# GestaltCogTeam/STEP

Measured on AMD Instinct MI355X. Metric: training windows/sec on PEMS04, horizon-12 MAE parity, 1/2/4/8 MI355X, higher is better.
Workload: dtype f16 (TSFormer Q/K/weights) + bf16 (P, V, GraphWaveNet / graph-learner GEMMs) operands, f32 accumulate

## Files before the change

step_amd/build.py:

```python
import os
import subprocess
import sys

HERE = os.path.dirname(os.path.abspath(__file__))
CSRC = os.path.join(HERE, "csrc")
LIB = os.path.join(HERE, "libstep_hip.so")
SOURCES = ["errors.cpp", "comm.cpp", "gemm.hip", "gemm_bf16.hip", "tsformer_encoder.hip", "knn.hip", "selftest.hip",
           "dgl.hip", "dgl_conv_mfma.hip", "gwnet.hip", "optim.hip", "pretrain.hip", "pretrain_fused.hip", "pretrain_attn2.hip",
           "eval_cache.hip", "eval_metrics.hip", "train_tail.hip"]


def _newer(target, deps):
    if not os.path.exists(target):
        return True
    t = os.path.getmtime(target)
    return any(os.path.getmtime(d) > t for d in deps)


def build(force=False, verbose=True):
    hipcc = os.environ.get("HIPCC", "/opt/rocm/bin/hipcc")
    srcs = [os.path.join(CSRC, s) for s in SOURCES if os.path.exists(os.path.join(CSRC, s))]
    hdrs = [os.path.join(CSRC, f) for f in os.listdir(CSRC) if f.endswith(".h")]
    hdrs.append(os.path.join(HERE, "..", "include", "step_hip.h"))
    objs = []
    os.makedirs(os.path.join(HERE, "build"), exist_ok=True)
    procs = []
    for s in srcs:
        o = os.path.join(HERE, "build", os.path.basename(s) + ".o")
        objs.append(o)
        if force or _newer(o, [s] + hdrs):
            cmd = [hipcc, "--offload-arch=gfx950", "-O3", "-std=c++17", "-fPIC", "-x", "hip", "-c", s, "-o", o]
            if verbose:
                print(" ".join(cmd), flush=True)
            procs.append((s, subprocess.Popen(cmd, stdout=subprocess.PIPE, stderr=subprocess.STDOUT)))
    for s, p in procs:
        out, _ = p.communicate()
        if p.returncode != 0:
            sys.stderr.write(out.decode())
            raise RuntimeError("hipcc failed on " + s)
    if force or _newer(LIB, objs):
        cmd = [hipcc, "--offload-arch=gfx950", "-shared", "-fPIC", "-o", LIB] + objs + ["-ldl"]
        if verbose:
            print(" ".join(cmd), flush=True)
        subprocess.check_call(cmd)
    return LIB


if __name__ == "__main__":
    build(force="--force" in sys.argv)
```

step_amd/csrc/dgl.hip:

```cpp
#include "common.h"
#include "step_internal.h"

namespace {

constexpr int KW = 10;
constexpr int EMB = 100;

template <int CI, int CO, int TPT>
__global__ __launch_bounds__(256) void conv_relu_fwd_kernel(const float* __restrict__ in, const float* __restrict__ w,
                                                            const float* __restrict__ b, const float* __restrict__ in_sc,
                                                            const float* __restrict__ in_sh, float* __restrict__ out,
                                                            float* __restrict__ partial, int Tin, int stat_limit) {
    __shared__ __attribute__((aligned(16))) float ws[CI * KW * CO];
    __shared__ float red[4][2 * CO];
    const int tid = threadIdx.x, n = blockIdx.y;
    const int Tout = Tin - (KW - 1);
    for (int e = tid; e < CI * KW * CO; e += 256) {
        int co = e % CO, k = (e / CO) % KW, ci = e / (CO * KW);
        ws[e] = w[(co * CI + ci) * KW + k];
    }
    __syncthreads();
    const int t0 = (blockIdx.x * 256 + tid) * TPT;
    float acc[CO][TPT];
#pragma unroll
// ... 512 lines not shown
    if (tid < EMB) {
        drcv[(long)i * EMB + tid] = ra[tid] * sw[tid];
        atomicAdd(&dwcat[tid], rh[tid]);
        atomicAdd(&dwcat[EMB + tid], -rh[tid]);
    }
    if (tid == 0) {
        const float s = red[0] + red[1] + red[2] + red[3];
        atomicAdd(&dbcat[0], s);
        atomicAdd(&dbcat[1], -s);
    }
}
template <int VJ>
__global__ __launch_bounds__(256) void edge_bwd_col_kernel(const float* __restrict__ dz, const float* __restrict__ sndT,
                                                           const float* __restrict__ rcv, const float* __restrict__ wcat, int N,
                                                           float* __restrict__ dsndT) {
    const int lane = threadIdx.x & 63, wave = threadIdx.x >> 6;
    const int j = (blockIdx.x * 64 + lane) * VJ;
    const int f = blockIdx.y * 4 + wave;
    if (j >= N || f >= EMB) return;
    const float wd = wcat[f] - wcat[EMB + f];
    if constexpr (VJ == 4) {
        const float4 s4 = *(const float4*)(sndT + (long)f * N + j);
        float a0 = 0.f, a1 = 0.f, a2 = 0.f, a3 = 0.f;
#pragma unroll 8
        for (int i = 0; i < N; ++i) {
            const float r = rcv[(long)i * EMB + f];
            const float4 d = *(const float4*)(dz + (long)i * N + j);
            a0 += r + s4.x > 0.f ? d.x : 0.f; a1 += r + s4.y > 0.f ? d.y : 0.f;
            a2 += r + s4.z > 0.f ? d.z : 0.f; a3 += r + s4.w > 0.f ? d.w : 0.f;
        }
        *(float4*)(dsndT + (long)f * N + j) = make_float4(a0 * wd, a1 * wd, a2 * wd, a3 * wd);
    } else {
        const float s = sndT[(long)f * N + j];
        float a = 0.f;
#pragma unroll 8
        for (int i = 0; i < N; ++i) {
            float hid = rcv[(long)i * EMB + f] + s;
            float d = dz[(long)i * N + j];
            a += hid > 0.f ? d : 0.f;
        }
        dsndT[(long)f * N + j] = a * wd;
    }
}

__global__ void colsum_kernel(const float* __restrict__ x, long rows, int cols, long ld, float* __restrict__ out) {
    __shared__ float red[4][64];
    const int c = blockIdx.x * 64 + (threadIdx.x & 63);
    const int w = threadIdx.x >> 6;
    float s = 0.f;
    if (c < cols)
        for (long r = (long)blockIdx.y * 4 + w; r < rows; r += (long)gridDim.y * 4) s += x[r * ld + c];
    red[w][threadIdx.x & 63] = s;
    __syncthreads();
    if (w == 0 && c < cols) atomicAdd(&out[c], red[0][threadIdx.x] + red[1][threadIdx.x] + red[2][threadIdx.x] + red[3][threadIdx.x]);
}

}

int step_colsum_launch(const float* x, long rows, int cols, long ld, float* out, hipStream_t st) {
    int chunks = (int)((rows + 255) / 256);
    if (chunks > 512) chunks = 512;
    if (chunks < 1) chunks = 1;
    colsum_kernel<<<dim3(cdiv(cols, 64), chunks), 256, 0, st>>>(x, rows, cols, ld, out);
    STEP_LAUNCH_CHECK("colsum");
    return STEP_OK;
}

constexpr int DGL_SMALL = 256 + 64 + 1344 + 100 * 32;

__global__ void bn2_fused_coef_kernel(const float* __restrict__ dots, const float* __restrict__ stat, const float* __restrict__ gamma,
                                      double count, float* __restrict__ dgamma, float* __restrict__ dbeta, float* __restrict__ coef) {
    constexpr int C = 16;
    const int c = threadIdx.x;
    if (c >= C) return;
    const float S1 = dots[2 * c + 1];
    const float S2 = stat[3 * C + c] * (dots[2 * c] - stat[2 * C + c] * S1);
    dgamma[c] += S2;
    dbeta[c] += S1;
    coef[c] = (float)(S1 / count);
    coef[C + c] = (float)(S2 / count);
    coef[2 * C + c] = gamma[c] * stat[3 * C + c];
}

__global__ __launch_bounds__(256) void fc_prep_kernel(const float* __restrict__ fc_w, const float* __restrict__ st2, uint4* __restrict__ wp,
                                                      float* __restrict__ shiftdot, int T2) {
    __shared__ float red[4];
    const int o = blockIdx.y, t = blockIdx.x * 256 + threadIdx.x, tid = threadIdx.x;
    float acc = 0.f;
    if (t < T2) {
        float v[16];
#pragma unroll
        for (int c = 0; c < 16; ++c) v[c] = fc_w[((long)o * 16 + c) * T2 + t];
#pragma unroll
        for (int c = 0; c < 16; ++c) { acc += v[c] * st2[16 + c]; v[c] *= st2[c]; }
        uint4* dst = wp + ((long)o * T2 + t) * 2;
        dst[0] = make_uint4(pack_bf16x2(v[0], v[1]), pack_bf16x2(v[2], v[3]), pack_bf16x2(v[4], v[5]), pack_bf16x2(v[6], v[7]));
        dst[1] = make_uint4(pack_bf16x2(v[8], v[9]), pack_bf16x2(v[10], v[11]), pack_bf16x2(v[12], v[13]), pack_bf16x2(v[14], v[15]));
    }
    acc = wave_sum(acc);
    if ((tid & 63) == 0) red[tid >> 6] = acc;
    __syncthreads();
    if (tid == 0) atomicAdd(&shiftdot[o], red[0] + red[1] + red[2] + red[3]);
}
__global__ void gpre_init_kernel(float* __restrict__ gpre, const float* __restrict__ shiftdot, long n) {
    const long i = (long)blockIdx.x * 256 + threadIdx.x;
    if (i < n) gpre[i] = shiftdot[i % EMB];
}
__global__ __launch_bounds__(256) void fc_unpermute_kernel(const float* __restrict__ graw, const float* __restrict__ fc_w,
                                                           const float* __restrict__ st2, const float* __restrict__ colsum,
                                                           float* __restrict__ dfc_w, float* __restrict__ dots_o, int T2, int overwrite) {
    __shared__ float red[4][32];
    const int o = blockIdx.y, t = blockIdx.x * 256 + threadIdx.x, tid = threadIdx.x;
    const float cso = colsum[o];
    float d[32];
#pragma unroll
    for (int i = 0; i < 32; ++i) d[i] = 0.f;
    if (t < T2) {
        const float4* src = (const float4*)(graw + ((long)o * T2 + t) * 16);
        const float4 g0 = src[0], g1 = src[1], g2 = src[2], g3 = src[3];
        const float g[16] = {g0.x, g0.y, g0.z, g0.w, g1.x, g1.y, g1.z, g1.w, g2.x, g2.y, g2.z, g2.w, g3.x, g3.y, g3.z, g3.w};
        float w[16], old[16];
#pragma unroll
        for (int c = 0; c < 16; ++c) { const long idx = ((long)o * 16 + c) * T2 + t; w[c] = fc_w[idx]; old[c] = overwrite ? 0.f : dfc_w[idx]; }
#pragma unroll
        for (int c = 0; c < 16; ++c) {
            dfc_w[((long)o * 16 + c) * T2 + t] = old[c] + st2[c] * g[c] + st2[16 + c] * cso;
            d[2 * c] = w[c] * g[c]; d[2 * c + 1] = w[c] * cso;
        }
    }
#pragma unroll
    for (int i = 0; i < 32; ++i) {
        const float v = wave_sum(d[i]);
        if ((tid & 63) == 0) red[tid >> 6][i] = v;
    }
    __syncthreads();
    if (tid < 32) atomicAdd(&dots_o[o * 32 + tid], red[0][tid] + red[1][tid] + red[2][tid] + red[3][tid]);
}
__global__ void dots_reduce_kernel(const float* __restrict__ dots_o, float* __restrict__ dots) {
    const int i = threadIdx.x;
    if (i >= 32) return;
    double a = 0.0;
    for (int o = 0; o < EMB; ++o) a += dots_o[o * 32 + i];
    dots[i] = (float)a;
}

static bool dgl_channels_last(const StepDglParams* p) {
    const char* e = getenv("STEP_DGL_F32_STORAGE");
    return p->gemm_bf16 && !(e && e[0] == '1');
}

static bool dgl_legacy_bn_backward() {
    const char* e = getenv("STEP_DGL_LEGACY_BN");
    return e && e[0] == '1';
}

extern "C" long step_dgl_global_saved_floats(int N, int T) {
    long T1 = T - 9, T2 = T - 18;
    return (long)N * 8 * T1 + (long)N * 16 * T2 + (long)N * EMB + 4 * 8 + 4 * 16 + 4 * EMB + (long)EMB * 16 * T2 + 128;
}
static long fc_splitk_ws_floats(int N, int T2) {
    const int splits = step_gemm_auto_splitk(N, EMB, 16 * T2, 1);
    return splits > 1 ? (long)splits * N * EMB + 4 : 0;
}
extern "C" long step_dgl_global_work_floats(int N, int T, int backward) {
    long T1 = T - 9, T2 = T - 18;
    long nb1 = (long)N * cdiv(T1, 1024), nb2 = (long)N * cdiv(T2, 1024);
    long part = (nb1 > nb2 ? nb1 : nb2) * 32 + 64;
    if (!backward) return part + dgl_conv2_pack_floats() + 64 + fc_splitk_ws_floats(N, (int)T2);
    return part + (long)N * 16 * T2 + (long)N * 8 * T1 + (long)EMB * 16 * T2 + 2L * N * EMB + DGL_SMALL + dgl_conv2_wgrad_scratch_floats(N, (int)T1);
}

static float* saved_wp(float* saved, int N, int T) {
    long T1 = T - 9, T2 = T - 18;
    return saved + (long)N * 8 * T1 + (long)N * 16 * T2 + (long)N * EMB + 4 * 8 + 4 * 16 + 4 * EMB;
}
static void carve_saved(float* saved, int N, int T, float** a1, float** a2, float** gpre, float** st1, float** st2, float** st3) {
    long T1 = T - 9, T2 = T - 18;
    *a1 = saved; saved += (long)N * 8 * T1;
    *a2 = saved; saved += (long)N * 16 * T2;
    *gpre = saved; saved += (long)N * EMB;
    *st1 = saved; saved += 4 * 8;
    *st2 = saved; saved += 4 * 16;
    *st3 = saved;
}

static int dgl_bn_stats(const float* partial, int nblk, int C, double count, const float* gamma, const float* beta, float* rm, float* rv,
                        int training, float momentum, float* stat, double* sums, hipStream_t st) {
    if (nblk < 8192) {
        bn_finalize_kernel<<<C, 256, 0, st>>>(partial, nblk, C, count, gamma, beta, rm, rv, training, momentum, stat);
    } else {
        if (hipMemsetAsync(sums, 0, 2 * C * sizeof(double), st) != hipSuccess) { step_set_error("memset failed"); return STEP_ERR_HIP; }
        bn_sums_sliced_kernel<<<dim3(C, 32), 256, 0, st>>>(partial, nblk, C, sums);
        bn_finalize_sums_kernel<<<1, 64, 0, st>>>(sums, C, count, gamma, beta, rm, rv, training, momentum, stat);
    }
    STEP_LAUNCH_CHECK("bn_stats");
    return STEP_OK;
}

static int dgl_global_forward_impl(const float* series_nt, int N, int T, const StepDglParams* p, int training, float momentum,
                                   float* saved, float* work, double* sums, float* g, const StepDglShard* shard, int phase,
                                   hipStream_t st) {
    const int T1 = T - 9, T2 = T - 18;
    float *a1, *a2, *gpre, *st1, *st2, *st3;
    carve_saved(saved, N, T, &a1, &a2, &gpre, &st1, &st2, &st3);
    float* partial = work;
    const bool all = phase == 0;
    const double count1 = shard ? shard->count1 : (double)N * T1, count2 = shard ? shard->count2 : (double)N * T2;
    const bool cl = dgl_channels_last(p);
    const long part_floats = ((long)N * cdiv(T1, 1024) > (long)N * cdiv(T2, 1024) ? (long)N * cdiv(T1, 1024) : (long)N * cdiv(T2, 1024)) * 32 + 64;
    double* own_sums = (double*)(work + part_floats + dgl_conv2_pack_floats());
    float* wp = saved_wp(saved, N, T);
    float* shiftdot = wp + (long)EMB * 16 * T2;
    if (all || phase == 1) {
        int nblk;
        if (cl) {
            STEP_TRY(dgl_conv1_fwd_cl(series_nt, p->conv1_w, p->conv1_b, a1, partial, N, T, shard ? shard->own1 : T1, &nblk, st));
        } else {
            dim3 grid(cdiv(T1, 256 * 4), N);
            conv_relu_fwd_kernel<1, 8, 4><<<grid, 256, 0, st>>>(series_nt, p->conv1_w, p->conv1_b, nullptr, nullptr, a1, partial, T,
                                                                shard ? shard->own1 : T1);
            STEP_LAUNCH_CHECK("conv1");
            nblk = grid.x * grid.y;
        }
        if (shard) bn_sums_kernel<<<8, 256, 0, st>>>(partial, nblk, 8, sums);
        else STEP_TRY(dgl_bn_stats(partial, nblk, 8, count1, p->bn1_w, p->bn1_b, p->bn1_rm, p->bn1_rv, training, momentum, st1, own_sums, st));
        STEP_LAUNCH_CHECK("bn1");
    }
    if (all || phase == 2) {
        if (shard) bn_finalize_sums_kernel<<<1, 64, 0, st>>>(sums, 8, count1, p->bn1_w, p->bn1_b, p->bn1_rm, p->bn1_rv, training, momentum, st1);
        int nblk;
        if (cl) {
            STEP_TRY(dgl_conv2_fwd_cl(a1, p->conv2_w, p->conv2_b, st1, st1 + 8, a2, partial, N, T1, &nblk,
                                      work + part_floats, st));
        } else if (p->gemm_bf16) {
            STEP_TRY(dgl_conv2_fwd_mfma(a1, p->conv2_w, p->conv2_b, st1, st1 + 8, a2, partial, N, T1, &nblk, st));
        } else {
            dim3 grid(cdiv(T2, 256 * 4), N);
            conv_relu_fwd_kernel<8, 16, 4><<<grid, 256, 0, st>>>(a1, p->conv2_w, p->conv2_b, st1, st1 + 8, a2, partial, T1, T2);
            STEP_LAUNCH_CHECK("conv2");
            nblk = grid.x * grid.y;
        }
        if (shard) bn_sums_kernel<<<16, 256, 0, st>>>(partial, nblk, 16, sums + 16);
        else STEP_TRY(dgl_bn_stats(partial, nblk, 16, count2, p->bn2_w, p->bn2_b, p->bn2_rm, p->bn2_rv, training, momentum, st2, own_sums, st));
        STEP_LAUNCH_CHECK("bn2");
    }
    if (all || phase == 3) {
        if (shard) bn_finalize_sums_kernel<<<1, 64, 0, st>>>(sums + 16, 16, count2, p->bn2_w, p->bn2_b, p->bn2_rm, p->bn2_rv, training, momentum, st2);
        const long K = 16L * T2;
        StepGemm gm = gemm_desc(N, EMB, (int)K, a2, K, 1, p->fc_w, 1, K, gpre, EMB);
        if (cl) {
            if (hipMemsetAsync(shiftdot, 0, 128 * sizeof(float), st) != hipSuccess) { step_set_error("memset failed"); return STEP_ERR_HIP; }
            fc_prep_kernel<<<dim3(cdiv(T2, 256), EMB), 256, 0, st>>>(p->fc_w, st2, (uint4*)wp, shiftdot, T2);
            gpre_init_kernel<<<cdiv((long)N * EMB, 256), 256, 0, st>>>(gpre, shiftdot, (long)N * EMB);
            STEP_LAUNCH_CHECK("fc_prep");
            gm.a_bf16 = 1;
            gm.B = wp; gm.b_bf16 = 1;
        } else {
            if (hipMemsetAsync(gpre, 0, (size_t)N * EMB * sizeof(float), st) != hipSuccess) { step_set_error("memset failed"); return STEP_ERR_HIP; }
            gm.a_kscale = st2; gm.a_kshift = st2 + 16; gm.a_kperiod = T2;
        }
        gm.accumulate = 2;
        gm.splitk = -1;
        gm.compute_bf16 = p->gemm_bf16;
        if (fc_splitk_ws_floats(N, T2) > 0) {
            float* ws = work + part_floats + dgl_conv2_pack_floats() + 64;
            gm.splitk_ws = (float*)(((uintptr_t)ws + 15) & ~(uintptr_t)15);
            gm.splitk_ws_floats = fc_splitk_ws_floats(N, T2) - 4;
        }
        STEP_TRY(step_gemm_launch(gm, st));
    }
    if (all || phase == 4) {
        fc_post_bn3_kernel<<<EMB, 256, 0, st>>>(gpre, p->fc_b, N, p->bn3_w, p->bn3_b, p->bn3_rm, p->bn3_rv, training, momentum, st3, g);
        STEP_LAUNCH_CHECK("fc_post_bn3");
    }
    return STEP_OK;
}

extern "C" int step_dgl_global_forward(const float* series_nt, int N, int T, const StepDglParams* p, int training,
                                       float momentum, float* saved, float* work, float* g, void* stream) {
    STEP_REQUIRE(series_nt && p && saved && work && g && N > 0 && T > 18, "dgl_global_forward: bad arguments");
    return dgl_global_forward_impl(series_nt, N, T, p, training, momentum, saved, work, nullptr, g, nullptr, 0, (hipStream_t)stream);
}

extern "C" int step_dgl_global_forward_shard(const float* series_slice, int N, int Ts, const StepDglParams* p, int training,
                                             float momentum, float* saved, float* work, double* sums, float* g,
                                             const StepDglShard* shard, int phase, void* stream) {
    STEP_REQUIRE(series_slice && p && saved && work && sums && g && shard && N > 0 && Ts > 18 && phase >= 1 && phase <= 4,
                 "dgl_global_forward_shard: bad arguments");
    STEP_REQUIRE(shard->own1 > 0 && shard->own1 <= Ts - 9 && shard->count1 > 0 && shard->count2 > 0, "dgl_global_forward_shard: bad shard");
    return dgl_global_forward_impl(series_slice, N, Ts, p, training, momentum, saved, work, sums, g, shard, phase, (hipStream_t)stream);
}

extern "C" long step_dgl_global_offset(int N, int T, int item) {
    const long T1 = T - 9, T2 = T - 18;
    if (item == 0) return 0;
    if (item == 1) return (long)N * 8 * T1;
    if (item == 2) return (long)N * 8 * T1 + (long)N * 16 * T2;
    const long nb1 = (long)N * cdiv(T1, 1024), nb2 = (long)N * cdiv(T2, 1024);
    const long coef = (nb1 > nb2 ? nb1 : nb2) * 32 + 64 + (long)N * 16 * T2 + (long)N * 8 * T1 + (long)EMB * 16 * T2 + 2L * N * EMB;
    if (item == 10) return coef + 256;
    if (item == 11) return coef + 320;
    return -1;
}

static int dgl_global_backward_impl(const float* series_nt, int N, int T, const StepDglParams* p, const float* saved, const float* dg,
                                    float* work, const StepDglParams* grads, const StepDglShard* shard, int phase, void* stream);

extern "C" int step_dgl_global_backward(const float* series_nt, int N, int T, const StepDglParams* p, const float* saved,
                                        const float* dg, float* work, const StepDglParams* grads, void* stream) {
    return step_dgl_global_backward_phase(series_nt, N, T, p, saved, dg, work, grads, 0, stream);
}

extern "C" int step_dgl_global_backward_phase(const float* series_nt, int N, int T, const StepDglParams* p, const float* saved,
                                              const float* dg, float* work, const StepDglParams* grads, int phase, void* stream) {
    STEP_REQUIRE(series_nt && p && saved && dg && work && grads && N > 0 && T > 18 && (phase & ~STEP_DGL_FRESH_FC_GRAD) >= 0 &&
                 (phase & ~STEP_DGL_FRESH_FC_GRAD) <= 2, "dgl_global_backward: bad arguments");
    return dgl_global_backward_impl(series_nt, N, T, p, saved, dg, work, grads, nullptr, phase, stream);
}

extern "C" int step_dgl_global_backward_shard(const float* series_slice, int N, int Ts, const StepDglParams* p, const float* saved,
                                              const float* dg, float* work, const StepDglParams* grads, const StepDglShard* shard,
                                              int phase, void* stream) {
    const int ph = phase & ~STEP_DGL_FRESH_FC_GRAD;
    STEP_REQUIRE(series_slice && p && saved && dg && work && grads && shard && N > 0 && Ts > 18 && (ph == 1 || ph == 3 || ph == 4),
                 "dgl_global_backward_shard: bad arguments");
    STEP_REQUIRE(p->gemm_bf16 && Ts - 18 >= 128, "dgl_global_backward_shard: needs the bf16 contraction mode and a slice of >= 128 conv2 columns");
    return dgl_global_backward_impl(series_slice, N, Ts, p, saved, dg, work, grads, shard, phase, stream);
}

static int dgl_global_backward_impl(const float* series_nt, int N, int T, const StepDglParams* p, const float* saved, const float* dg,
                                    float* work, const StepDglParams* grads, const StepDglShard* shard, int phase, void* stream) {
    const int fresh_fc = (phase & STEP_DGL_FRESH_FC_GRAD) ? 1 : 0;
    phase &= ~STEP_DGL_FRESH_FC_GRAD;
    const bool do_fc = phase == 0 || phase == 1, do_mid = phase == 0 || phase == 2 || phase == 3, do_tail = phase == 0 || phase == 2 || phase == 4;
    hipStream_t st = (hipStream_t)stream;
    const int T1 = T - 9, T2 = T - 18;
    const long K = 16L * T2;
    float *a1, *a2, *gpre, *st1, *st2, *st3;
    carve_saved((float*)saved, N, T, &a1, &a2, &gpre, &st1, &st2, &st3);
    long nb1 = (long)N * cdiv(T1, 1024), nb2 = (long)N * cdiv(T2, 1024);
    float* partial = work;
    float* d_a2 = work + (nb1 > nb2 ? nb1 : nb2) * 32 + 64;
    float* d_a1 = d_a2 + (long)N * 16 * T2;
    float* wraw = d_a1 + (long)N * 8 * T1;
    float* dgpre = wraw + (long)EMB * K;
    float* dgpreT = dgpre + (long)N * EMB;
    float* coef = dgpreT + (long)N * EMB;
    float* dots = coef + 256;
    float* graw = coef + 320;
    float* wg_scratch = coef + DGL_SMALL;
    const bool fuse2 = T2 >= 128 && (shard || !dgl_legacy_bn_backward());
    const double count1 = shard ? shard->count1 : (double)N * T1, count2 = shard ? shard->count2 : (double)N * T2;
    if (dgl_channels_last(p)) {
        const float* wp = saved_wp((float*)saved, N, T);
        float* dots_o = coef + 256 + 64 + 1344;
        float* colsum = coef + 128;
        if (do_fc) {
            bn3_relu_bwd_kernel<<<EMB, 256, 0, st>>>(dg, gpre, N, p->bn3_w, st3, grads->bn3_w, grads->bn3_b, grads->fc_b, dgpre, dgpreT, colsum);
            STEP_LAUNCH_CHECK("bn3_bwd");
            StepGemm gm = gemm_desc(EMB, (int)K, N, dgpre, 1, EMB, a2, K, 1, wraw, K);
            gm.b_bf16 = 1;
            gm.compute_bf16 = 1;
            STEP_TRY(step_gemm_launch(gm, st));
            if (hipMemsetAsync(dots_o, 0, EMB * 32 * sizeof(float), st) != hipSuccess) { step_set_error("memset failed"); return STEP_ERR_HIP; }
            fc_unpermute_kernel<<<dim3(cdiv(T2, 256), EMB), 256, 0, st>>>(wraw, p->fc_w, st2, colsum, grads->fc_w, dots_o, T2, fresh_fc);
            dots_reduce_kernel<<<1, 64, 0, st>>>(dots_o, dots);
            STEP_LAUNCH_CHECK("fc_unpermute");
        }
        if (do_mid) {
            bn2_fused_coef_kernel<<<1, 64, 0, st>>>(dots, st2, p->bn2_w, count2, grads->bn2_w, grads->bn2_b, coef);
            STEP_LAUNCH_CHECK("bn2_fused_coef");
            StepGemm gm = gemm_desc(N, (int)K, EMB, dgpre, EMB, 1, wp, K, 1, d_a2, K);
            gm.b_bf16 = 1;
            gm.compute_bf16 = 1;
            GemmFused fu = {nullptr, nullptr, a2, coef, st2, 16, T2, GEMM_FUSED_INTERLEAVED};
            STEP_TRY(step_gemm_launch_fused(gm, fu, st));
            STEP_TRY(dgl_conv2_wgrad_cl(d_a2, a1, wg_scratch, graw, N, T1, st));
        }
        if (do_tail) {
            STEP_TRY(dgl_conv2_wgrad_finish(graw, p->conv2_w, st1, p->bn1_w, p->bn1_b, count1, grads->conv2_w, grads->conv2_b, grads->bn1_w,
                                            grads->bn1_b, coef + 64, 1, st));
            STEP_TRY(dgl_conv2_dgrad_cl(d_a2, p->conv2_w, st1, d_a1, N, T1, a1, coef + 64, st1, shard ? shard->own1 : T1, wraw, st));
            STEP_TRY(dgl_conv1_wgrad_cl(d_a1, series_nt, wg_scratch, grads->conv1_w, grads->conv1_b, N, T, st));
        }
        return STEP_OK;
    }
    if (do_fc) {
        float* colsum = coef + 128;
        bn3_relu_bwd_kernel<<<EMB, 256, 0, st>>>(dg, gpre, N, p->bn3_w, st3, grads->bn3_w, grads->bn3_b, grads->fc_b, dgpre, dgpreT, colsum);
        STEP_LAUNCH_CHECK("bn3_bwd");
        {
            StepGemm gm = gemm_desc(EMB, (int)K, N, dgpre, 1, EMB, a2, K, 1, grads->fc_w, K);
            gm.accumulate = fresh_fc ? 0 : 1;
            gm.c_nscale = st2; gm.c_nshift = st2 + 16; gm.c_nperiod = T2; gm.c_mvec = colsum;
            gm.compute_bf16 = p->gemm_bf16;
            if (fuse2) {
                if (hipMemsetAsync(dots, 0, 32 * sizeof(float), st) != hipSuccess) { step_set_error("memset failed"); return STEP_ERR_HIP; }
                GemmFused fu = {p->fc_w, dots, nullptr, nullptr, nullptr, 16, T2};
                STEP_TRY(step_gemm_launch_fused(gm, fu, st));
            } else {
                STEP_TRY(step_gemm_launch(gm, st));
            }
        }
    }
    if (!do_mid && !do_tail) return STEP_OK;
    if (do_mid) {
        StepGemm gm = gemm_desc(N, (int)K, EMB, dgpreT, 1, N, p->fc_w, K, 1, d_a2, K);
        if (p->gemm_bf16 || fuse2) { gm.A = dgpre; gm.sam = EMB; gm.sak = 1; }
        gm.compute_bf16 = p->gemm_bf16;
        if (fuse2) {
            bn2_fused_coef_kernel<<<1, 64, 0, st>>>(dots, st2, p->bn2_w, count2, grads->bn2_w, grads->bn2_b, coef);
            STEP_LAUNCH_CHECK("bn2_fused_coef");
            GemmFused fu = {nullptr, nullptr, a2, coef, st2, 16, T2};
            STEP_TRY(step_gemm_launch_fused(gm, fu, st));
        } else {
            STEP_TRY(step_gemm_launch(gm, st));
        }
    }
    if (do_mid && !fuse2) {
        dim3 grid(cdiv(T2, 1024), 16, N);
        bn_bwd_reduce_kernel<16><<<grid, 256, 0, st>>>(d_a2, a2, st2, T2, partial);
        STEP_LAUNCH_CHECK("bn2_bwd_reduce");
        bn_bwd_finalize_kernel<<<16, 256, 0, st>>>(partial, (int)nb2, 16, (double)N * T2, p->bn2_w, st2, grads->bn2_w, grads->bn2_b, coef);
        STEP_LAUNCH_CHECK("bn2_bwd_finalize");
        bn_bwd_apply_kernel<16><<<grid, 256, 0, st>>>(d_a2, a2, st2, coef, T2);
        STEP_LAUNCH_CHECK("bn2_bwd_apply");
    }
    const bool fuse1 = p->gemm_bf16 && (shard || !dgl_legacy_bn_backward());
    if (fuse1) {
        if (do_mid) STEP_TRY(dgl_conv2_wgrad_xhat_mfma(d_a2, a1, st1, wg_scratch, graw, N, T1, st));
        if (!do_tail) return STEP_OK;
        STEP_TRY(dgl_conv2_wgrad_finish(graw, p->conv2_w, st1, p->bn1_w, p->bn1_b, count1, grads->conv2_w, grads->conv2_b, grads->bn1_w,
                                        grads->bn1_b, coef + 64, 0, st));
        STEP_TRY(dgl_conv2_dgrad_mfma(d_a2, p->conv2_w, d_a1, N, T1, a1, coef + 64, st1, shard ? shard->own1 : T1, st));
    } else if (p->gemm_bf16) {
        STEP_TRY(dgl_conv2_wgrad_mfma(d_a2, a1, st1, st1 + 8, wg_scratch, grads->conv2_w, grads->conv2_b, N, T1, st));
        STEP_TRY(dgl_conv2_dgrad_mfma(d_a2, p->conv2_w, d_a1, N, T1, nullptr, nullptr, nullptr, T1, st));
    } else {
        conv_bwd_weight_kernel<8, 16><<<N, 256, 0, st>>>(d_a2, a1, st1, st1 + 8, grads->conv2_w, grads->conv2_b, T1);
        STEP_LAUNCH_CHECK("conv2_bwd_weight");
        conv_bwd_data_kernel<8, 16, 4><<<dim3(cdiv(T1, 1024), N), 256, 0, st>>>(d_a2, p->conv2_w, d_a1, T1);
        STEP_LAUNCH_CHECK("conv2_bwd_data");
    }
    if (!fuse1) {
        dim3 grid(cdiv(T1, 1024), 8, N);
        bn_bwd_reduce_kernel<8><<<grid, 256, 0, st>>>(d_a1, a1, st1, T1, partial);
        STEP_LAUNCH_CHECK("bn1_bwd_reduce");
        bn_bwd_finalize_kernel<<<8, 256, 0, st>>>(partial, (int)nb1, 8, (double)N * T1, p->bn1_w, st1, grads->bn1_w, grads->bn1_b, coef);
        STEP_LAUNCH_CHECK("bn1_bwd_finalize");
        bn_bwd_apply_kernel<8><<<grid, 256, 0, st>>>(d_a1, a1, st1, coef, T1);
        STEP_LAUNCH_CHECK("bn1_bwd_apply");
    }
    if (p->gemm_bf16) {
        STEP_TRY(dgl_conv1_wgrad_mfma(d_a1, series_nt, wg_scratch, grads->conv1_w, grads->conv1_b, N, T, st));
    } else {
        conv_bwd_weight_kernel<1, 8><<<N, 256, 0, st>>>(d_a1, series_nt, nullptr, nullptr, grads->conv1_w, grads->conv1_b, T);
        STEP_LAUNCH_CHECK("conv1_bwd_weight");
    }
    return STEP_OK;
}

extern "C" long step_dgl_edges_saved_floats(int B, int N) { return 2L * N * EMB + (long)N * N + 2L * B * N * N; }
extern "C" long step_dgl_edges_theta_offset(int N) { return 2L * N * EMB + (long)N * N; }

extern "C" int step_dgl_edges_forward(const float* g, int N, int B, const StepDglParams* p, const float* u, uint64_t seed,
                                      float temperature, float* saved, float* theta_out, float* adj_out, void* stream) {
    return step_dgl_edges_forward_dyn(g, N, B, p, u, seed, temperature, saved, theta_out, adj_out, nullptr, stream);
}
extern "C" int step_dgl_edges_forward_dyn(const float* g, int N, int B, const StepDglParams* p, const float* u, uint64_t seed,
                                          float temperature, float* saved, float* theta_out, float* adj_out, const StepDynState* dyn,
                                          void* stream) {
    STEP_REQUIRE(g && p && saved && adj_out && N > 0 && B > 0 && temperature > 0.f, "dgl_edges_forward: bad arguments");
    hipStream_t st = (hipStream_t)stream;
    float* sndT = saved;
    float* rcv = sndT + (long)N * EMB;
    float* z = rcv + (long)N * EMB;
    float* theta = z + (long)N * N;
    float* y0 = theta + (long)B * N * N;
    StepGemm gs = gemm_desc(N, EMB, EMB, g, EMB, 1, p->fc_out_w, 1, 2 * EMB, sndT, 1);
    gs.scn = N;
    STEP_TRY(step_gemm_launch(gs, st));
    StepGemm gr = gemm_desc(N, EMB, EMB, g, EMB, 1, p->fc_out_w + EMB, 1, 2 * EMB, rcv, EMB);
    gr.bias = p->fc_out_b;
    STEP_TRY(step_gemm_launch(gr, st));
    {
        const int vec4 = N % 4 == 0 && N >= 1024 && (((uintptr_t)sndT | (uintptr_t)z) & 15) == 0;
        edge_logit_kernel<<<dim3(cdiv(N, vec4 ? 1024 : 256), N), 256, 0, st>>>(sndT, rcv, p->fc_cat_w, p->fc_cat_b, N, z, vec4);
    }
    STEP_LAUNCH_CHECK("edge_logit");
    int gx = cdiv((long)N * N, 256);
    if (gx > 4096) gx = 4096;
    gumbel_sample_kernel<<<dim3(gx, B), 256, 0, st>>>(z, u, B, N, (uint32_t)seed, (uint32_t)(seed >> 32), 1.f / temperature, theta, y0, adj_out, dyn);
    STEP_LAUNCH_CHECK("gumbel_sample");
    if (theta_out && theta_out != theta) {
        if (hipMemcpyAsync(theta_out, theta, (size_t)B * N * N * sizeof(float), hipMemcpyDeviceToDevice, st) != hipSuccess) {
            step_set_error("dgl_edges_forward: theta copy failed");
            return STEP_ERR_HIP;
        }
    }
    return STEP_OK;
}

extern "C" long step_dgl_edges_work_floats(int N) { return (long)N * N + 2L * N * EMB; }

extern "C" int step_dgl_edges_backward(const float* g, int N, int B, const StepDglParams* p, const float* saved,
                                       const float* dtheta, const float* dadj, float temperature, float* work,
                                       const StepDglParams* grads, float* dg, void* aux_stream, void* stream) {
    STEP_REQUIRE(g && p && saved && work && grads && dg && N > 0 && B > 0, "dgl_edges_backward: bad arguments");
    hipStream_t st = (hipStream_t)stream;
    AuxLane lane(st, (hipStream_t)aux_stream);
    const float* sndT = saved;
    const float* rcv = sndT + (long)N * EMB;
    const float* theta = rcv + (long)N * EMB + (long)N * N;
    const float* y0 = theta + (long)B * N * N;
    float* dz = work;
    float* drcv = dz + (long)N * N;
    float* dsndT = drcv + (long)N * EMB;
    int gx = cdiv((long)N * N, 256);
    if (gx > 4096) gx = 4096;
    edge_dz_kernel<<<gx, 256, 0, st>>>(dtheta, dadj, theta, y0, B, N, 1.f / temperature, dz);
// ... 25 lines not shown
```

step_amd/csrc/step_internal.h:

```cpp
#pragma once
#include <hip/hip_runtime.h>
#include <vector>
#include "../../include/step_hip.h"

enum { GEMM_FUSED_INTERLEAVED = 1, GEMM_FUSED_FFN_FWD = 2, GEMM_FUSED_MASKNZ = 4, GEMM_FUSED_BF16OUT = 8 };
struct GemmFused {
    const float* dotw; float* dots;
    const float* bnx; const float* bncoef; const float* bnstat;
    int channels, period;
    int flags;
    const float* ffn_bias; const void* maskx; float p; unsigned seed_lo, seed_hi, site;
};

struct GemmKSeg { long a_off, b_off, a_bs, b_bs; int a_rs, b_rs; };
constexpr int GEMM_KSEG_MAX = 128;
int step_gemm_segmented_launch(StepGemm g, const GemmKSeg* ktab, int ktab_per, hipStream_t st);

int step_gemm_launch(StepGemm g, hipStream_t st);
int step_gemm_auto_splitk(int M, int N, int K, int batch);
int step_gemm_launch_fused(StepGemm g, const GemmFused& fused, hipStream_t st);
int step_gemm_bf16_launch(StepGemm g, hipStream_t st, const GemmFused* fused = nullptr);
int step_gemm_f32_fast_launch(StepGemm g, hipStream_t st, const GemmFused* fused = nullptr);

static inline StepGemm gemm_desc(int M, int N, int K, const float* A, long sam, long sak, const float* B, long sbk,
                                 long sbn, float* C, long ldc) {
    StepGemm g;
    memset(&g, 0, sizeof(g));
    g.M = M; g.N = N; g.K = K; g.batch = 1;
    g.A = A; g.sam = sam; g.sak = sak;
    g.B = B; g.sbk = sbk; g.sbn = sbn;
    g.C = C; g.ldc = ldc; g.scn = 1;
    g.alpha = 1.f; g.splitk = 1;
    return g;
}

int step_gemm_rowsum_separate(StepGemm* g, hipStream_t st);
int dgl_conv2_fwd_mfma(const float* a1, const float* w, const float* b, const float* sc, const float* sh, float* a2, float* partial,
                       int N, int T1, int* nblk, hipStream_t st);
int dgl_conv2_dgrad_mfma(const float* dz, const float* w, float* din, int N, int T1, const float* bnx, const float* coef, const float* stat,
                         int own, hipStream_t st);
int dgl_conv2_wgrad_xhat_mfma(const float* dz, const float* a1, const float* stat1, float* scratch, float* graw, int N, int T1, hipStream_t st);
int dgl_conv2_wgrad_finish(const float* graw, const float* w, const float* stat1, const float* gamma1, const float* beta1, double count,
                           float* dw, float* db, float* dgamma1, float* dbeta1, float* coef1, int raw, hipStream_t st);
int dgl_conv1_fwd_cl(const float* x, const float* w, const float* b, void* a1h, float* partial, int N, int T, int stat_limit, int* nblk,
                     hipStream_t st);
long dgl_conv2_pack_floats();
int dgl_conv2_fwd_cl(const void* a1h, const float* w, const float* b, const float* sc, const float* sh, void* a2h, float* partial, int N,
                     int T1, int* nblk, float* pack, hipStream_t st);
int dgl_conv2_dgrad_cl(const void* dz2h, const float* w, const float* sc, void* dz1h, int N, int T1, const void* a1h, const float* coef,
                       const float* stat, int own, float* pack, hipStream_t st);
int dgl_conv2_wgrad_cl(const void* dz2h, const void* a1h, float* scratch, float* graw, int N, int T1, hipStream_t st);
int dgl_conv1_wgrad_cl(const void* dz1h, const float* x, float* scratch, float* dw, float* db, int N, int T, hipStream_t st);
long dgl_conv2_wgrad_scratch_floats(int N, int T1);
int dgl_conv2_wgrad_mfma(const float* dz, const float* a1, const float* sc, const float* sh, float* scratch, float* dw, float* db, int N,
                         int T1, hipStream_t st);
int dgl_conv1_wgrad_mfma(const float* dz, const float* x, float* scratch, float* dw, float* db, int N, int T, hipStream_t st);
int step_colsum_launch(const float* x, long rows, int cols, long ld, float* out, hipStream_t st);

struct AuxLane {
    hipStream_t main, aux;
    bool on;
    int next = 0, base = 0;
    AuxLane(hipStream_t m, hipStream_t a, int base_ = 0) : main(m), aux(a), on(a != nullptr && a != m), base(base_) {}
    static hipEvent_t event(int k) {
        thread_local std::vector<hipEvent_t> pool[16];
        int dev = 0;
        (void)hipGetDevice(&dev);
        std::vector<hipEvent_t>& v = pool[dev & 15];
        while ((int)v.size() <= k) {
            hipEvent_t e;
            if (hipEventCreateWithFlags(&e, hipEventDisableTiming) != hipSuccess) return nullptr;
            v.push_back(e);
        }
        return v[k];
    }
    hipStream_t fork() {
        if (!on) return main;
        hipEvent_t e = event(base + (next++ & 63));
        if (!e || hipEventRecord(e, main) != hipSuccess || hipStreamWaitEvent(aux, e, 0) != hipSuccess) { on = false; return main; }
        return aux;
    }
    hipEvent_t mark() {
        if (!on) return nullptr;
        hipEvent_t e = event(base + (next++ & 63));
        if (!e || hipEventRecord(e, main) != hipSuccess) { on = false; return nullptr; }
        return e;
    }
    hipStream_t after(hipEvent_t e) {
        if (!on || !e) return main;
        if (hipStreamWaitEvent(aux, e, 0) != hipSuccess) { on = false; return main; }
        return aux;
    }
    hipEvent_t done() {
        if (!on) return nullptr;
        hipEvent_t e = event(base + (next++ & 63));
        if (!e || hipEventRecord(e, aux) != hipSuccess) return nullptr;
        return e;
    }
    int wait_done(hipEvent_t e) {
        if (!on) return STEP_OK;
        if (!e) return join();
        if (hipStreamWaitEvent(main, e, 0) != hipSuccess) { step_set_error("backward: stream join failed"); return STEP_ERR_HIP; }
        return STEP_OK;
    }
    int join() {
        if (!on) return STEP_OK;
        hipEvent_t e = event(base + (next++ & 63));
        if (!e || hipEventRecord(e, aux) != hipSuccess || hipStreamWaitEvent(main, e, 0) != hipSuccess) {
            step_set_error("backward: stream join failed");
            return STEP_ERR_HIP;
        }
        return STEP_OK;
    }
};
```

Before: 2358.

## Fuse graph-learner FC weight-gradient GEMM with unpermute and BN dot reduction

Adds a dedicated MFMA kernel for the graph-learner FC weight gradient. Its epilogue applies the BN2 scale/shift, writes dfc_w in the original layout and produces the per-channel dot partials in one pass. This replaces the generic GEMM, the raw-gradient buffer round trip, the unpermute kernel and the memset. It also adds an opt-in fused forward kernel that folds the weight pack/scale into a split-K MFMA GEMM. The forward path stays behind an environment flag, while the backward fused path is on by default. The cost is a new hand-written kernel, and the per-block LDS and partial workspace (passed via wraw) need to be large enough.

```diff
diff --git a/step_amd/build.py b/step_amd/build.py
--- a/step_amd/build.py
+++ b/step_amd/build.py
@@ -6,7 +6,7 @@
 CSRC = os.path.join(HERE, "csrc")
 LIB = os.path.join(HERE, "libstep_hip.so")
 SOURCES = ["errors.cpp", "comm.cpp", "gemm.hip", "gemm_bf16.hip", "tsformer_encoder.hip", "knn.hip", "selftest.hip",
-           "dgl.hip", "dgl_conv_mfma.hip", "gwnet.hip", "optim.hip", "pretrain.hip", "pretrain_fused.hip", "pretrain_attn2.hip",
+           "dgl.hip", "dgl_fc.hip", "dgl_conv_mfma.hip", "gwnet.hip", "optim.hip", "pretrain.hip", "pretrain_fused.hip", "pretrain_attn2.hip",
            "eval_cache.hip", "eval_metrics.hip", "train_tail.hip"]
 
 
diff --git a/step_amd/csrc/dgl.hip b/step_amd/csrc/dgl.hip
--- a/step_amd/csrc/dgl.hip
+++ b/step_amd/csrc/dgl.hip
@@ -688,6 +688,15 @@
 static bool dgl_legacy_bn_backward() {
     const char* e = getenv("STEP_DGL_LEGACY_BN");
     return e && e[0] == '1';
+}
+
+static bool dgl_fc_staged() {
+    const char* e = getenv("STEP_DGL_FC_STAGED");
+    return e && e[0] == '1';
+}
+static bool dgl_fc_fwd_fused() {
+    const char* e = getenv("STEP_DGL_FC_FWD_FUSED");
+    return e && e[0] == '1' && !dgl_fc_staged();
 }
 
 extern "C" long step_dgl_global_saved_floats(int N, int T) {
@@ -783,27 +792,35 @@
     if (all || phase == 3) {
         if (shard) bn_finalize_sums_kernel<<<1, 64, 0, st>>>(sums + 16, 16, count2, p->bn2_w, p->bn2_b, p->bn2_rm, p->bn2_rv, training, momentum, st2);
         const long K = 16L * T2;
-        StepGemm gm = gemm_desc(N, EMB, (int)K, a2, K, 1, p->fc_w, 1, K, gpre, EMB);
-        if (cl) {
-            if (hipMemsetAsync(shiftdot, 0, 128 * sizeof(float), st) != hipSuccess) { step_set_error("memset failed"); return STEP_ERR_HIP; }
-            fc_prep_kernel<<<dim3(cdiv(T2, 256), EMB), 256, 0, st>>>(p->fc_w, st2, (uint4*)wp, shiftdot, T2);
-            gpre_init_kernel<<<cdiv((long)N * EMB, 256), 256, 0, st>>>(gpre, shiftdot, (long)N * EMB);
-            STEP_LAUNCH_CHECK("fc_prep");
-            gm.a_bf16 = 1;
-            gm.B = wp; gm.b_bf16 = 1;
+        if (cl && dgl_fc_fwd_fused() && dgl_fc_fwd_cl_ok(N, a2, wp)) {
+            const int splits = step_gemm_auto_splitk(N, EMB, (int)K, 1), ksteps = cdiv(K, 64);
+            const int tper = 4 * cdiv(ksteps, splits > 1 ? splits : 1);
+            float* ws = work + part_floats + dgl_conv2_pack_floats() + 64;
+            ws = (float*)(((uintptr_t)ws + 15) & ~(uintptr_t)15);
+            STEP_TRY(dgl_fc_fwd_cl(a2, p->fc_w, st2, wp, ws, gpre, N, T2, tper, st));
         } else {
-            if (hipMemsetAsync(gpre, 0, (size_t)N * EMB * sizeof(float), st) != hipSuccess) { step_set_error("memset failed"); return STEP_ERR_HIP; }
-            gm.a_kscale = st2; gm.a_kshift = st2 + 16; gm.a_kperiod = T2;
-        }
-        gm.accumulate = 2;
-        gm.splitk = -1;
-        gm.compute_bf16 = p->gemm_bf16;
-        if (fc_splitk_ws_floats(N, T2) > 0) {
-            float* ws = work + part_floats + dgl_conv2_pack_floats() + 64;
-            gm.splitk_ws = (float*)(((uintptr_t)ws + 15) & ~(uintptr_t)15);
-            gm.splitk_ws_floats = fc_splitk_ws_floats(N, T2) - 4;
-        }
-        STEP_TRY(step_gemm_launch(gm, st));
+            StepGemm gm = gemm_desc(N, EMB, (int)K, a2, K, 1, p->fc_w, 1, K, gpre, EMB);
+            if (cl) {
+                if (hipMemsetAsync(shiftdot, 0, 128 * sizeof(float), st) != hipSuccess) { step_set_error("memset failed"); return STEP_ERR_HIP; }
+                fc_prep_kernel<<<dim3(cdiv(T2, 256), EMB), 256, 0, st>>>(p->fc_w, st2, (uint4*)wp, shiftdot, T2);
+                gpre_init_kernel<<<cdiv((long)N * EMB, 256), 256, 0, st>>>(gpre, shiftdot, (long)N * EMB);
+                STEP_LAUNCH_CHECK("fc_prep");
+                gm.a_bf16 = 1;
+                gm.B = wp; gm.b_bf16 = 1;
+            } else {
+                if (hipMemsetAsync(gpre, 0, (size_t)N * EMB * sizeof(float), st) != hipSuccess) { step_set_error("memset failed"); return STEP_ERR_HIP; }
+                gm.a_kscale = st2; gm.a_kshift = st2 + 16; gm.a_kperiod = T2;
+            }
+            gm.accumulate = 2;
+            gm.splitk = -1;
+            gm.compute_bf16 = p->gemm_bf16;
+            if (fc_splitk_ws_floats(N, T2) > 0) {
+                float* ws = work + part_floats + dgl_conv2_pack_floats() + 64;
+                gm.splitk_ws = (float*)(((uintptr_t)ws + 15) & ~(uintptr_t)15);
+                gm.splitk_ws_floats = fc_splitk_ws_floats(N, T2) - 4;
+            }
+            STEP_TRY(step_gemm_launch(gm, st));
+        }
     }
     if (all || phase == 4) {
         fc_post_bn3_kernel<<<EMB, 256, 0, st>>>(gpre, p->fc_b, N, p->bn3_w, p->bn3_b, p->bn3_rm, p->bn3_rv, training, momentum, st3, g);
@@ -894,14 +911,18 @@
         if (do_fc) {
             bn3_relu_bwd_kernel<<<EMB, 256, 0, st>>>(dg, gpre, N, p->bn3_w, st3, grads->bn3_w, grads->bn3_b, grads->fc_b, dgpre, dgpreT, colsum);
             STEP_LAUNCH_CHECK("bn3_bwd");
-            StepGemm gm = gemm_desc(EMB, (int)K, N, dgpre, 1, EMB, a2, K, 1, wraw, K);
-            gm.b_bf16 = 1;
-            gm.compute_bf16 = 1;
-            STEP_TRY(step_gemm_launch(gm, st));
-            if (hipMemsetAsync(dots_o, 0, EMB * 32 * sizeof(float), st) != hipSuccess) { step_set_error("memset failed"); return STEP_ERR_HIP; }
-            fc_unpermute_kernel<<<dim3(cdiv(T2, 256), EMB), 256, 0, st>>>(wraw, p->fc_w, st2, colsum, grads->fc_w, dots_o, T2, fresh_fc);
-            dots_reduce_kernel<<<1, 64, 0, st>>>(dots_o, dots);
-            STEP_LAUNCH_CHECK("fc_unpermute");
+            if (!dgl_fc_staged()) {
+                STEP_TRY(dgl_fc_wgrad_cl(dgpre, a2, p->fc_w, st2, colsum, grads->fc_w, wraw, dots, N, T2, fresh_fc, st));
+            } else {
+                StepGemm gm = gemm_desc(EMB, (int)K, N, dgpre, 1, EMB, a2, K, 1, wraw, K);
+                gm.b_bf16 = 1;
+                gm.compute_bf16 = 1;
+                STEP_TRY(step_gemm_launch(gm, st));
+                if (hipMemsetAsync(dots_o, 0, EMB * 32 * sizeof(float), st) != hipSuccess) { step_set_error("memset failed"); return STEP_ERR_HIP; }
+                fc_unpermute_kernel<<<dim3(cdiv(T2, 256), EMB), 256, 0, st>>>(wraw, p->fc_w, st2, colsum, grads->fc_w, dots_o, T2, fresh_fc);
+                dots_reduce_kernel<<<1, 64, 0, st>>>(dots_o, dots);
+                STEP_LAUNCH_CHECK("fc_unpermute");
+            }
         }
         if (do_mid) {
             bn2_fused_coef_kernel<<<1, 64, 0, st>>>(dots, st2, p->bn2_w, count2, grads->bn2_w, grads->bn2_b, coef);
diff --git a/step_amd/csrc/dgl_fc.hip b/step_amd/csrc/dgl_fc.hip
--- /dev/null
+++ b/step_amd/csrc/dgl_fc.hip
@@ -0,0 +1,307 @@
+#include "common.h"
+#include "step_internal.h"
+
+namespace {
+
+constexpr int EMB = 100;
+constexpr int WG_TB = 32, WG_COLS = WG_TB * 16;
+constexpr int WG_KT = 32;
+constexpr int WG_PITCH = WG_KT * 2 + 16;
+constexpr int WG_ABUF = 128 * WG_PITCH, WG_BUF = WG_ABUF + WG_COLS * WG_PITCH;
+constexpr int WG_LDS = 2 * WG_BUF;
+constexpr int WG_CP = 36, WG_RP = 16 * WG_CP + 4;
+static_assert(32 * WG_RP * 4 <= WG_LDS, "epilogue tile must fit in the operand buffers");
+
+__global__ __launch_bounds__(512) void fc_wgrad_cl_kernel(const float* __restrict__ dgpre, const uint16_t* __restrict__ a2h,
+                                                          const float* __restrict__ fc_w, const float* __restrict__ st2,
+                                                          const float* __restrict__ colsum, float* __restrict__ dfc_w,
+                                                          float* __restrict__ part, int N, int T2, int overwrite) {
+    extern __shared__ __attribute__((aligned(16))) char wl[];
+    const int tid = threadIdx.x, lane = tid & 63, wave = tid >> 6, r = lane & 31, h = lane >> 5;
+    const int t0 = blockIdx.x * WG_TB;
+    const long K = 16L * T2;
+
+    f32x16 acc[4][2];
+#pragma unroll
+    for (int i = 0; i < 4; ++i)
+#pragma unroll
+        for (int j = 0; j < 2; ++j)
+#pragma unroll
+            for (int e = 0; e < 16; ++e) acc[i][j][e] = 0.f;
+
+    const int ao = tid & 127, akq = tid >> 7;
+    const long bcol = (long)t0 * 16 + 8 * lane;
+    const bool bcol_ok = bcol < K;
+    float av[8];
+    uint32_t bw[4][4];
+    auto fetch = [&](int kt) {
+#pragma unroll
+        for (int j = 0; j < 8; ++j) {
+            const int n = kt * WG_KT + akq * 8 + j;
+            av[j] = (ao < EMB && n < N) ? dgpre[(long)n * EMB + ao] : 0.f;
+        }
+#pragma unroll
+        for (int j = 0; j < 4; ++j) {
+            const int n = kt * WG_KT + wave * 4 + j;
+            uint4 v = make_uint4(0u, 0u, 0u, 0u);
+            if (bcol_ok && n < N) v = *(const uint4*)(a2h + (long)n * K + bcol);
+            bw[j][0] = v.x; bw[j][1] = v.y; bw[j][2] = v.z; bw[j][3] = v.w;
+        }
+    };
+    auto commit = [&](char* buf) {
+        *(bf16x8*)(buf + ao * WG_PITCH + akq * 16) = pack8(av);
+        char* d = buf + WG_ABUF + lane * WG_PITCH + wave * 8;
+#pragma unroll
+        for (int p = 0; p < 4; ++p) {
+            const uint32_t d0 = bw[0][p], d1 = bw[1][p], d2 = bw[2][p], d3 = bw[3][p];
+            *(uint2*)(d + (2 * p) * 64 * WG_PITCH) = make_uint2((d0 & 0xffffu) | (d1 << 16), (d2 & 0xffffu) | (d3 << 16));
+            *(uint2*)(d + (2 * p + 1) * 64 * WG_PITCH) = make_uint2((d0 >> 16) | (d1 & 0xffff0000u), (d2 >> 16) | (d3 & 0xffff0000u));
+        }
+    };
+
+    const int nkt = 2 * ((N + 63) / 64);
+    fetch(0);
+    commit(wl);
+    __syncthreads();
+    int cur = 0;
+    for (int kt = 0; kt < nkt; ++kt) {
+        const bool more = kt + 1 < nkt;
+        if (more) fetch(kt + 1);
+        const char* As = wl + cur * WG_BUF;
+        const char* Bs = As + WG_ABUF + (2 * wave * 32 + r) * WG_PITCH;
+#pragma unroll
+        for (int ks = 0; ks < WG_KT / 16; ++ks) {
+            bf16x8 a[4], b[2];
+#pragma unroll
+            for (int i = 0; i < 4; ++i) a[i] = *(const bf16x8*)(As + (i * 32 + r) * WG_PITCH + ks * 32 + h * 16);
+#pragma unroll
+            for (int j = 0; j < 2; ++j) b[j] = *(const bf16x8*)(Bs + j * 32 * WG_PITCH + ks * 32 + h * 16);
+#pragma unroll
+            for (int i = 0; i < 4; ++i)
+#pragma unroll
+                for (int j = 0; j < 2; ++j) acc[i][j] = __builtin_amdgcn_mfma_f32_32x32x16_bf16(a[i], b[j], acc[i][j], 0, 0, 0);
+        }
+        if (more) commit(wl + (cur ^ 1) * WG_BUF);
+        __syncthreads();
+        cur ^= 1;
+    }
+
+    float* tile = (float*)wl;
+    const int tl = tid & 31, c = tid >> 5, t = t0 + tl;
+    const bool tok = t < T2;
+    const float sc = st2[c], sh = st2[16 + c];
+    float dw = 0.f, dm = 0.f;
+#pragma unroll
+    for (int i = 0; i < 4; ++i) {
+#pragma unroll
+        for (int j = 0; j < 2; ++j) {
+            float* q = tile + (8 * (r & 1) + wave) * WG_CP + j * 16 + (r >> 1) + 4 * h * WG_RP;
+#pragma unroll
+            for (int e = 0; e < 16; ++e) q[((e & 3) + 8 * (e >> 2)) * WG_RP] = acc[i][j][e];
+        }
+        __syncthreads();
+        const int rows = EMB - i * 32 < 32 ? EMB - i * 32 : 32;
+        for (int ol0 = 0; ol0 < rows; ol0 += 8) {
+            float w8[8], o8[8];
+            long idx[8];
+            bool ok[8];
+#pragma unroll
+            for (int u = 0; u < 8; ++u) {
+                const int o = i * 32 + ol0 + u;
+                ok[u] = tok && o < EMB;
+                idx[u] = ok[u] ? ((long)o * 16 + c) * T2 + t : 0;
+                w8[u] = fc_w[idx[u]];
+                o8[u] = overwrite ? 0.f : dfc_w[idx[u]];
+            }
+#pragma unroll
+            for (int u = 0; u < 8; ++u) {
+                if (!ok[u]) continue;
+                const float g = tile[(ol0 + u) * WG_RP + c * WG_CP + tl];
+                const float cso = colsum[i * 32 + ol0 + u];
+                dfc_w[idx[u]] = fmaf(sh, cso, fmaf(sc, g, o8[u]));
+                dw = fmaf(w8[u], g, dw);
+                dm = fmaf(w8[u], cso, dm);
+            }
+        }
+        __syncthreads();
+    }
+#pragma unroll
+    for (int o = 16; o > 0; o >>= 1) { dw += __shfl_xor(dw, o, 64); dm += __shfl_xor(dm, o, 64); }
+    if (tl == 0) { part[(long)blockIdx.x * 32 + 2 * c] = dw; part[(long)blockIdx.x * 32 + 2 * c + 1] = dm; }
+}
+
+__global__ __launch_bounds__(256) void fc_dots_reduce_kernel(const float* __restrict__ part, int rows, float* __restrict__ dots) {
+    __shared__ double red[8][32];
+    const int col = threadIdx.x & 31, s = threadIdx.x >> 5;
+    double a = 0.0;
+    for (int row = s; row < rows; row += 8) a += part[(long)row * 32 + col];
+    red[s][col] = a;
+    __syncthreads();
+    if (threadIdx.x < 32) {
+        double v = 0.0;
+#pragma unroll
+        for (int k = 0; k < 8; ++k) v += red[k][col];
+        dots[col] = (float)v;
+    }
+}
+
+constexpr int FW_WAVES = 10, FW_THREADS = FW_WAVES * 64;
+constexpr int FW_ROWB = 128;
+constexpr int FW_ABUF = FW_WAVES * 32 * FW_ROWB, FW_BUF = FW_ABUF + 128 * FW_ROWB;
+constexpr int FW_LDS = 2 * FW_BUF;
+constexpr int FW_NA = FW_WAVES * 32 * 8 / FW_THREADS, FW_NB = (128 * 8 + FW_THREADS - 1) / FW_THREADS;
+
+__global__ __launch_bounds__(FW_THREADS) void fc_fwd_cl_kernel(const uint16_t* __restrict__ a2h, const float* __restrict__ fc_w,
+                                                               const float* __restrict__ st2, uint16_t* wp, float* __restrict__ ws, int N,
+                                                               int T2, int tper) {
+    extern __shared__ __attribute__((aligned(16))) char fl[];
+    __shared__ float sd[128];
+    const int tid = threadIdx.x, lane = tid & 63, wave = tid >> 6, r = lane & 31, h = lane >> 5;
+    const long K = 16L * T2;
+    const int ts0 = blockIdx.x * tper, ts1 = min(T2, ts0 + tper);
+    const long kbeg = 16L * ts0, kend = 16L * ts1;
+
+    {
+        float sc[16], sh[16];
+#pragma unroll
+        for (int c = 0; c < 16; ++c) { sc[c] = st2[c]; sh[c] = st2[16 + c]; }
+        if (tid >= EMB && tid < 128) sd[tid] = 0.f;
+        for (int o = wave; o < EMB; o += FW_WAVES) {
+            float acc = 0.f;
+            for (int tb = ts0; tb < ts1; tb += 64) {
+                const int t = tb + lane;
+                if (t < ts1) {
+                    float v[16];
+#pragma unroll
+                    for (int c = 0; c < 16; ++c) v[c] = fc_w[((long)o * 16 + c) * T2 + t];
+#pragma unroll
+                    for (int c = 0; c < 16; ++c) { acc += v[c] * sh[c]; v[c] *= sc[c]; }
+                    uint4* dst = (uint4*)(wp + ((long)o * T2 + t) * 16);
+                    dst[0] = make_uint4(pack_bf16x2(v[0], v[1]), pack_bf16x2(v[2], v[3]), pack_bf16x2(v[4], v[5]), pack_bf16x2(v[6], v[7]));
+                    dst[1] = make_uint4(pack_bf16x2(v[8], v[9]), pack_bf16x2(v[10], v[11]), pack_bf16x2(v[12], v[13]), pack_bf16x2(v[14], v[15]));
+                }
+            }
+            acc = wave_sum(acc);
+            if (lane == 0) sd[o] = acc;
+        }
+        __threadfence();
+        __syncthreads();
+    }
+
+    f32x16 acc[4];
+#pragma unroll
+    for (int j = 0; j < 4; ++j)
+#pragma unroll
+        for (int e = 0; e < 16; ++e) acc[j][e] = 0.f;
+
+    uint4 ra[FW_NA], rb[FW_NB];
+    const uint16_t* wpr = wp;
+    auto fetch = [&](long k0) {
+#pragma unroll
+        for (int j = 0; j < FW_NA; ++j) {
+            const int e = tid + j * FW_THREADS;
+            int row = e >> 3;
+            const long k = k0 + (e & 7) * 8;
+            row = row < N ? row : N - 1;
+            ra[j] = make_uint4(0u, 0u, 0u, 0u);
+            if (k < kend) ra[j] = *(const uint4*)(a2h + (long)row * K + k);
+        }
+#pragma unroll
+        for (int j = 0; j < FW_NB; ++j) {
+            const int e = tid + j * FW_THREADS;
+            const int row = e >> 3;
+            const long k = k0 + (e & 7) * 8;
+            rb[j] = make_uint4(0u, 0u, 0u, 0u);
+            if (row < EMB && k < kend) rb[j] = *(const uint4*)(wpr + (long)row * K + k);
+        }
+    };
+    auto commit = [&](char* buf) {
+#pragma unroll
+        for (int j = 0; j < FW_NA; ++j) {
+            const int e = tid + j * FW_THREADS, row = e >> 3;
+            *(uint4*)(buf + row * FW_ROWB + (((e & 7) ^ (row & 7)) << 4)) = ra[j];
+        }
+#pragma unroll
+        for (int j = 0; j < FW_NB; ++j) {
+            const int e = tid + j * FW_THREADS, row = e >> 3;
+            if (e < 128 * 8) *(uint4*)(buf + FW_ABUF + row * FW_ROWB + (((e & 7) ^ (row & 7)) << 4)) = rb[j];
+        }
+    };
+
+    const int nslab = (int)((kend - kbeg + 63) / 64);
+    fetch(kbeg);
+    commit(fl);
+    __syncthreads();
+    int cur = 0;
+    for (int s = 0; s < nslab; ++s) {
+        const bool more = s + 1 < nslab;
+        if (more) fetch(kbeg + 64L * (s + 1));
+        const char* As = fl + cur * FW_BUF + (wave * 32 + r) * FW_ROWB;
+        const char* Bs = fl + cur * FW_BUF + FW_ABUF + r * FW_ROWB;
+#pragma unroll
+        for (int ks = 0; ks < 4; ++ks) {
+            const int sl = ((ks * 2 + h) ^ (r & 7)) << 4;
+            const bf16x8 a = *(const bf16x8*)(As + sl);
+#pragma unroll
+            for (int j = 0; j < 4; ++j) {
+                const bf16x8 b = *(const bf16x8*)(Bs + j * 32 * FW_ROWB + sl);
+                acc[j] = __builtin_amdgcn_mfma_f32_32x32x16_bf16(a, b, acc[j], 0, 0, 0);
+            }
+        }
+        if (more) commit(fl + (cur ^ 1) * FW_BUF);
+        __syncthreads();
+        cur ^= 1;
+    }
+
+    float* out = ws + (long)blockIdx.x * N * EMB;
+#pragma unroll
+    for (int j = 0; j < 4; ++j) {
+        const int o = j * 32 + r;
+        if (o >= EMB) continue;
+        const float sv = sd[o];
+#pragma unroll
+        for (int e = 0; e < 16; ++e) {
+            const int n = wave * 32 + 4 * h + (e & 3) + 8 * (e >> 2);
+            if (n < N) out[(long)n * EMB + o] = acc[j][e] + sv;
+        }
+    }
+}
+
+__global__ __launch_bounds__(256) void fc_reduce_kernel(const float* __restrict__ ws, int nsl, long mn, float* __restrict__ gpre) {
+    const long i = (long)blockIdx.x * 256 + threadIdx.x;
+    if (i >= mn) return;
+    const float* src = ws + i;
+    float v0 = 0.f, v1 = 0.f, v2 = 0.f, v3 = 0.f;
+    int z = 0;
+    for (; z + 4 <= nsl; z += 4) { v0 += src[(long)z * mn]; v1 += src[(long)(z + 1) * mn]; v2 += src[(long)(z + 2) * mn]; v3 += src[(long)(z + 3) * mn]; }
+    for (; z < nsl; ++z) v0 += src[(long)z * mn];
+    gpre[i] = (v0 + v1) + (v2 + v3);
+}
+
+}
+
+bool dgl_fc_fwd_cl_ok(int N, const void* a2h, const void* wp) { return N <= FW_WAVES * 32 && (((uintptr_t)a2h | (uintptr_t)wp) & 15) == 0; }
+
+int dgl_fc_fwd_cl(const void* a2h, const float* fc_w, const float* st2, void* wp, float* ws, float* gpre, int N, int T2, int tper,
+                  hipStream_t st) {
+    STEP_REQUIRE(dgl_fc_fwd_cl_ok(N, a2h, wp) && tper > 0, "fc_fwd_cl: needs at most 320 nodes and 16-byte aligned bf16 rows");
+    if (step_raise_lds_once((const void*)fc_fwd_cl_kernel, FW_LDS, "fc_fwd_cl") != 0) return STEP_ERR_HIP;
+    const int nsl = cdiv(T2, tper);
+    fc_fwd_cl_kernel<<<nsl, FW_THREADS, FW_LDS, st>>>((const uint16_t*)a2h, fc_w, st2, (uint16_t*)wp, nsl > 1 ? ws : gpre, N, T2, tper);
+    if (nsl > 1) fc_reduce_kernel<<<cdiv((long)N * EMB, 256), 256, 0, st>>>(ws, nsl, (long)N * EMB, gpre);
+    STEP_LAUNCH_CHECK("fc_fwd_cl");
+    return STEP_OK;
+}
+
+long dgl_fc_wgrad_part_floats(int T2) { return 32L * cdiv(T2, WG_TB); }
+
+int dgl_fc_wgrad_cl(const float* dgpre, const void* a2h, const float* fc_w, const float* st2, const float* colsum, float* dfc_w, float* part,
+                    float* dots, int N, int T2, int overwrite, hipStream_t st) {
+    STEP_REQUIRE(((uintptr_t)a2h & 15) == 0, "fc_wgrad_cl: the bf16 activation rows must be 16-byte aligned");
+    if (step_raise_lds_once((const void*)fc_wgrad_cl_kernel, WG_LDS, "fc_wgrad_cl") != 0) return STEP_ERR_HIP;
+    const int nwg = cdiv(T2, WG_TB);
+    fc_wgrad_cl_kernel<<<nwg, 512, WG_LDS, st>>>(dgpre, (const uint16_t*)a2h, fc_w, st2, colsum, dfc_w, part, N, T2, overwrite);
+    fc_dots_reduce_kernel<<<1, 256, 0, st>>>(part, nwg, dots);
+    STEP_LAUNCH_CHECK("fc_wgrad_cl");
+    return STEP_OK;
+}
diff --git a/step_amd/csrc/step_internal.h b/step_amd/csrc/step_internal.h
--- a/step_amd/csrc/step_internal.h
+++ b/step_amd/csrc/step_internal.h
@@ -55,6 +55,12 @@
 int dgl_conv2_wgrad_mfma(const float* dz, const float* a1, const float* sc, const float* sh, float* scratch, float* dw, float* db, int N,
                          int T1, hipStream_t st);
 int dgl_conv1_wgrad_mfma(const float* dz, const float* x, float* scratch, float* dw, float* db, int N, int T, hipStream_t st);
+bool dgl_fc_fwd_cl_ok(int N, const void* a2h, const void* wp);
+int dgl_fc_fwd_cl(const void* a2h, const float* fc_w, const float* st2, void* wp, float* ws, float* gpre, int N, int T2, int tper,
+                  hipStream_t st);
+long dgl_fc_wgrad_part_floats(int T2);
+int dgl_fc_wgrad_cl(const float* dgpre, const void* a2h, const float* fc_w, const float* st2, const float* colsum, float* dfc_w, float* part,
+                    float* dots, int N, int T2, int overwrite, hipStream_t st);
 int step_colsum_launch(const float* x, long rows, int cols, long ld, float* out, hipStream_t st);
 
 struct AuxLane {
```

Measured after the change: 2362, median of 6. About the same (+0.2%).
